# nikopj/FlashAttention.jl

Measured on AMD Instinct MI355X. Metric: effective attention TFLOP/s (fwd) at N=4096,d=64; % of bf16 MFMA peak, higher is better.
Workload: dtype bf16; 1 GPU; configs[1]: dense_fa bf16 forward, (B,H,N,d)=(4,16,4096,64) per GPU; B=4, H=16, N=4096, d=64, slabs_per_gpu=64, global_batch_heads=64, parallelism=shard(B*H) x1, no collective

## Files before the change

### flashattention.jl_amd/csrc/fa_fwd.hip

```cpp
#include <type_traits>

#include "fa_common.h"
#include "fa_internal.h"
#include "fa_fwd_params.h"
#include "../../include/fa_hip.h"

#ifndef FA_FWD_STAMP
#define FA_FWD_STAMP(k)
#endif
#ifndef FA_FWD_ABL
#define FA_FWD_ABL 0
#endif
#ifndef FA_FWD_OAUX
#define FA_FWD_OAUX 0
#endif

namespace fa {

thread_local int g_fwd_variant = 0;
thread_local int g_fwd_last_path = 0;
thread_local float g_fwd_rescale_log2 = kRescaleLog2;


constexpr int kBM = 128;
constexpr int kBN = 64;
constexpr int kThreads = 256;

template <class T>
__device__ __forceinline__ u32x4 load_chunk(const T* base, int row, int col0, int nrows,
                                            int ncols, bool fast) {
    constexpr int EPC = 16 / sizeof(T);
    u32x4 z = {0u, 0u, 0u, 0u};
    if (row >= nrows) return z;
    const T* src = base + (int64_t)row * ncols;
    if (fast) {
        if (col0 >= ncols) return z;
        return *(const u32x4*)(src + col0);
    }
    union {
        T e[EPC];
        u32x4 v;
    } u;
#pragma unroll
    for (int e = 0; e < EPC; ++e) u.e[e] = (col0 + e < ncols) ? src[col0 + e] : (T)0.0f;
    return u.v;
}

template <class T, int D, int DV>
__global__ __launch_bounds__(kThreads) void dense_fwd_generic(FwdParams p) {
    typedef typename Frag8<T>::type F8;
    typedef typename Frag8<T>::half F4;
    constexpr int KROW = kBN * 2;
    constexpr int VROW = kBN * 2 + 16;
    constexpr int KCH = D * 8 / kThreads;
    constexpr int VCH = DV * 8 / kThreads;
    static_assert(KCH >= 1 && VCH >= 1, "head dim class too small");
    __shared__ __attribute__((aligned(16))) char smem[D * KROW + DV * VROW];
    char* const klds = smem;
    char* const vlds = smem + D * KROW;

    const int lid = xcd_remap(blockIdx.x, p.total_wg);
    const int b = lid / p.nqb;
    const int qb = lid - b * p.nqb;
    const int tid = threadIdx.x, lane = tid & 63, wave = tid >> 6;
    const int r = lane & 31, h = lane >> 5;
    const int N = p.N, Nk = p.Nk, d = p.d, dv = p.dv;
    const T* __restrict__ Qb = (const T*)p.Q + (int64_t)b * N * d;
    const T* __restrict__ Kb = (const T*)p.K + (int64_t)b * Nk * d;
    const T* __restrict__ Vb = (const T*)p.V + (int64_t)b * Nk * dv;
    const bool fast = p.fast != 0;

    const int qi = qb * kBM + wave * 32 + r;
    F8 qf[D / 16];
#pragma unroll
    for (int s = 0; s < D / 16; ++s)
#pragma unroll
        for (int e = 0; e < 8; ++e) {
            const int f = 16 * s + 8 * h + e;
            qf[s][e] = (qi < N && f < d) ? Qb[(int64_t)f * N + qi] : (T)0.0f;
        }

    const int g = lane >> 4, kh = g & 1, ii = lane & 15, qq = ii >> 2, pp = ii & 3;
    const int sig = (pp == 1) ? 2 : (pp == 2) ? 1 : pp;
    int koff[2];
#pragma unroll
    for (int kb = 0; kb < 2; ++kb)
        koff[kb] = (8 * h + qq) * KROW + (((kb * 2 + kh) ^ (((qq >> 1) & 1) << 1)) * 32) + 8 * sig;
    const int voff = r * VROW + 16 * h;

    f32x16 oacc[DV / 32];
#pragma unroll
    for (int cb = 0; cb < DV / 32; ++cb)
#pragma unroll
        for (int x = 0; x < 16; ++x) oacc[cb][x] = 0.0f;
    float m_run = kNegInf, l_run = 0.0f;
    const float c = p.scale_log2;

    u32x4 kreg[KCH], vreg[VCH];
    auto gload = [&](int j) {
        const int key0 = j * kBN;
#pragma unroll
        for (int it = 0; it < KCH; ++it) {
            const int ch = tid + kThreads * it;
            kreg[it] = load_chunk<T>(Kb, ch >> 3, key0 + (ch & 7) * 8, d, Nk, fast);
        }
#pragma unroll
        for (int it = 0; it < VCH; ++it) {
            const int ch = tid + kThreads * it;
            vreg[it] = load_chunk<T>(Vb, ch >> 3, key0 + (ch & 7) * 8, dv, Nk, fast);
        }
    };
    auto lstore = [&]() {
#pragma unroll
        for (int it = 0; it < KCH; ++it) {
            const int ch = tid + kThreads * it, f = ch >> 3, pc = ch & 7;
            const int off = f * KROW + (((pc >> 1) ^ (((f >> 1) & 1) << 1)) * 32) + (pc & 1) * 16;
            *(u32x4*)(klds + off) = kreg[it];
        }
#pragma unroll
        for (int it = 0; it < VCH; ++it) {
            const int ch = tid + kThreads * it;
            *(u32x4*)(vlds + (ch >> 3) * VROW + (ch & 7) * 16) = vreg[it];
        }
    };

    const int ntiles = (Nk + kBN - 1) / kBN;
    gload(0);
    lstore();
    __syncthreads();

    for (int j = 0; j < ntiles; ++j) {
        const bool more = j + 1 < ntiles;
        if (more) gload(j + 1);

        f32x16 sacc[2];
#pragma unroll
        for (int kb = 0; kb < 2; ++kb) {
#pragma unroll
            for (int x = 0; x < 16; ++x) sacc[kb][x] = 0.0f;
#pragma unroll
            for (int s = 0; s < D / 16; ++s) {
                const char* a = klds + koff[kb] + 16 * s * KROW;
                const F4 lo = __builtin_bit_cast(F4, ds_read_tr16(a));
                const F4 hi = __builtin_bit_cast(F4, ds_read_tr16(a + 4 * KROW));
                const F8 af = __builtin_shufflevector(lo, hi, 0, 1, 2, 3, 4, 5, 6, 7);
                sacc[kb] = mfma32x32x16(af, qf[s], sacc[kb]);
            }
        }

        const int key0 = j * kBN;
        if (key0 + kBN > Nk) {
#pragma unroll
            for (int kb = 0; kb < 2; ++kb)
#pragma unroll
                for (int x = 0; x < 16; ++x) {
                    const int kt = kb * 32 + (x & 3) + 4 * ((x >> 2) & 1) + 8 * h + 16 * (x >> 3);
                    if (key0 + kt >= Nk) sacc[kb][x] = kNegInf;
                }
        }

        float mt = kNegInf;
#pragma unroll
        for (int kb = 0; kb < 2; ++kb)
#pragma unroll
            for (int x = 0; x < 16; ++x) mt = fmaxf(mt, sacc[kb][x]);
        mt = swap_halves_max(mt);
        const float m_new = fmaxf(m_run, mt);
        const float alpha = exp2_fast((m_run - m_new) * c);
        const float mc = m_new * c;
        float ls = 0.0f;
        F8 pf[2][2];
#pragma unroll
        for (int kb = 0; kb < 2; ++kb)
#pragma unroll
            for (int x = 0; x < 16; ++x) {
                const float pv = exp2_fast(fmaf(sacc[kb][x], c, -mc));
                ls += pv;
                pf[kb][x >> 3][x & 7] = (T)pv;
            }
        l_run = l_run * alpha + ls;
        m_run = m_new;
#pragma unroll
        for (int cb = 0; cb < DV / 32; ++cb)
#pragma unroll
            for (int x = 0; x < 16; ++x) oacc[cb][x] *= alpha;

#pragma unroll
        for (int cb = 0; cb < DV / 32; ++cb)
#pragma unroll
            for (int kb = 0; kb < 2; ++kb)
#pragma unroll
                for (int s = 0; s < 2; ++s) {
                    const F8 va = *(const F8*)(vlds + voff + cb * 32 * VROW + (kb * 32 + 16 * s) * 2);
                    oacc[cb] = mfma32x32x16(va, pf[kb][s], oacc[cb]);
                }

        __syncthreads();
        if (more) {
            lstore();
            __syncthreads();
        }
    }

    const float lt = swap_halves_sum(l_run);
    const float inv = 1.0f / lt;
    if (qi < N) {
        T* Ob = (T*)p.O + (int64_t)b * N * dv;
#pragma unroll
        for (int cb = 0; cb < DV / 32; ++cb)
#pragma unroll
            for (int x = 0; x < 16; ++x) {
                const int cc = cb * 32 + acc_row(x, h);
                if (cc < dv) Ob[(int64_t)cc * N + qi] = (T)(oacc[cb][x] * inv);
            }
        if (h == 0) {
            p.m[(int64_t)b * N + qi] = m_run * p.scale;
            p.l[(int64_t)b * N + qi] = lt;
        }
    }
}

template <int D, int DV>
__global__ __launch_bounds__(kThreads) void dense_fwd_generic_f32(FwdParams p) {
    constexpr int KROWF = kBN;
    constexpr int VROWF = kBN + 1;
    constexpr int KCH = D * 16 / kThreads;
    constexpr int VCH = DV * 16 / kThreads;
    static_assert(KCH >= 1 && VCH >= 1, "head dim class too small");
    __shared__ __attribute__((aligned(16))) float smem[D * KROWF + DV * VROWF];
    float* const klds = smem;
    float* const vlds = smem + D * KROWF;

    const int lid = xcd_remap(blockIdx.x, p.total_wg);
    const int b = lid / p.nqb;
    const int qb = lid - b * p.nqb;
    const int tid = threadIdx.x, lane = tid & 63, wave = tid >> 6;
    const int r = lane & 31, h = lane >> 5;
    const int N = p.N, Nk = p.Nk, d = p.d, dv = p.dv;
    const float* __restrict__ Qb = (const float*)p.Q + (int64_t)b * N * d;
    const float* __restrict__ Kb = (const float*)p.K + (int64_t)b * Nk * d;
    const float* __restrict__ Vb = (const float*)p.V + (int64_t)b * Nk * dv;
    const bool fast = p.fast != 0;

    const int qi = qb * kBM + wave * 32 + r;
    float qf[D / 2];
#pragma unroll
    for (int t = 0; t < D / 2; ++t) {
        const int f = 2 * t + h;
        qf[t] = (qi < N && f < d) ? Qb[(int64_t)f * N + qi] : 0.0f;
    }

    f32x16 oacc[DV / 32];
#pragma unroll
    for (int cb = 0; cb < DV / 32; ++cb)
#pragma unroll
        for (int x = 0; x < 16; ++x) oacc[cb][x] = 0.0f;
    float m_run = kNegInf, l_run = 0.0f;
    const float c = p.scale_log2;

    u32x4 kreg[KCH], vreg[VCH];
    auto gload = [&](int j) {
        const int key0 = j * kBN;
#pragma unroll
        for (int it = 0; it < KCH; ++it) {
            const int ch = tid + kThreads * it;
            kreg[it] = load_chunk<float>(Kb, ch >> 4, key0 + (ch & 15) * 4, d, Nk, fast);
        }
#pragma unroll
        for (int it = 0; it < VCH; ++it) {
            const int ch = tid + kThreads * it;
            vreg[it] = load_chunk<float>(Vb, ch >> 4, key0 + (ch & 15) * 4, dv, Nk, fast);
        }
    };
    auto lstore = [&]() {
#pragma unroll
        for (int it = 0; it < KCH; ++it) {
            const int ch = tid + kThreads * it;
            *(u32x4*)(klds + (ch >> 4) * KROWF + (ch & 15) * 4) = kreg[it];
        }
#pragma unroll
        for (int it = 0; it < VCH; ++it) {
            const int ch = tid + kThreads * it;
            float* dst = vlds + (ch >> 4) * VROWF + (ch & 15) * 4;
#pragma unroll
            for (int e = 0; e < 4; ++e) dst[e] = __uint_as_float(vreg[it][e]);
        }
    };

    const int ntiles = (Nk + kBN - 1) / kBN;
    gload(0);
    lstore();
    __syncthreads();

    for (int j = 0; j < ntiles; ++j) {
        const bool more = j + 1 < ntiles;
        if (more) gload(j + 1);

        f32x16 sacc[2];
#pragma unroll
        for (int kb = 0; kb < 2; ++kb) {
#pragma unroll
            for (int x = 0; x < 16; ++x) sacc[kb][x] = 0.0f;
#pragma unroll
            for (int t = 0; t < D / 2; ++t)
                sacc[kb] = mfma32x32x2(klds[(2 * t + h) * KROWF + kb * 32 + r], qf[t], sacc[kb]);
        }

        const int key0 = j * kBN;
        if (key0 + kBN > Nk) {
#pragma unroll
            for (int kb = 0; kb < 2; ++kb)
#pragma unroll
                for (int x = 0; x < 16; ++x)
                    if (key0 + kb * 32 + acc_row(x, h) >= Nk) sacc[kb][x] = kNegInf;
        }

        float mt = kNegInf;
#pragma unroll
        for (int kb = 0; kb < 2; ++kb)
#pragma unroll
            for (int x = 0; x < 16; ++x) mt = fmaxf(mt, sacc[kb][x]);
        mt = swap_halves_max(mt);
        const float m_new = fmaxf(m_run, mt);
        const float alpha = exp2_fast((m_run - m_new) * c);
        const float mc = m_new * c;
        float ls = 0.0f;
#pragma unroll
        for (int kb = 0; kb < 2; ++kb)
#pragma unroll
            for (int x = 0; x < 16; ++x) {
                const float pv = exp2_fast(fmaf(sacc[kb][x], c, -mc));
                ls += pv;
                sacc[kb][x] = pv;
            }
        l_run = l_run * alpha + ls;
        m_run = m_new;
#pragma unroll
        for (int cb = 0; cb < DV / 32; ++cb)
#pragma unroll
            for (int x = 0; x < 16; ++x) oacc[cb][x] *= alpha;

#pragma unroll
        for (int cb = 0; cb < DV / 32; ++cb)
#pragma unroll
            for (int kb = 0; kb < 2; ++kb)
#pragma unroll
                for (int x = 0; x < 16; ++x)
                    oacc[cb] = mfma32x32x2(vlds[(cb * 32 + r) * VROWF + kb * 32 + acc_row(x, h)],
                                           sacc[kb][x], oacc[cb]);

        __syncthreads();
        if (more) {
            lstore();
            __syncthreads();
        }
    }

    const float lt = swap_halves_sum(l_run);
    const float inv = 1.0f / lt;
    if (qi < N) {
        float* Ob = (float*)p.O + (int64_t)b * N * dv;
#pragma unroll
        for (int cb = 0; cb < DV / 32; ++cb)
#pragma unroll
            for (int x = 0; x < 16; ++x) {
                const int cc = cb * 32 + acc_row(x, h);
                if (cc < dv) Ob[(int64_t)cc * N + qi] = oacc[cb][x] * inv;
            }
        if (h == 0) {
            p.m[(int64_t)b * N + qi] = m_run * p.scale;
            p.l[(int64_t)b * N + qi] = lt;
        }
    }
}


template <class T, int D, int DV, int NW, int BN, int NQB, bool SPLIT = false, bool WIDE = false>
__device__ __forceinline__ void dense_fwd_tiled(const FwdParams& p) {
    typedef typename Frag8<T>::type F8;
    typedef typename Frag8<T>::half F4;
    constexpr int NTH = 64 * NW;
    constexpr int BM = 32 * NW * NQB;
    constexpr int NKB = BN / 32;
    constexpr int KROW = BN * 2;
    constexpr int VROW = BN * 2 + 16;
    constexpr int KBYTES = D * KROW, VBYTES = DV * VROW, STAGE = KBYTES + VBYTES;
    constexpr int CPR = BN / 8;
    constexpr int KTOT = D * CPR, VTOT = DV * CPR;
    constexpr int KCH = (KTOT + NTH - 1) / NTH;
    constexpr int VCH = (VTOT + NTH - 1) / NTH;
    static_assert(KTOT % NTH == 0 || KTOT < NTH, "tile split");
    static_assert(VTOT % NTH == 0 || VTOT < NTH, "tile split");
    constexpr int ROWB = BM * 2;
    constexpr int QOOFF = (2 * STAGE + 16 + 255) & ~255;
    constexpr int QOB = WIDE ? (D > DV ? D : DV) * ROWB : 0;
    __shared__ __attribute__((aligned(256))) char smem[QOOFF + QOB];
    auto qo_at = [](int f, int byteoff) {
        const int X = (f & 3) | (((f >> 2) & 1) << 2);
        return f * ROWB + (((byteoff >> 5) ^ X) << 5) + (byteoff & 31);
    };
    char* const qoimg = smem + QOOFF;

    auto kswz = [](int f) { return BN == 64 ? (((f >> 1) & 1) << 1) : ((f & 3) << 1); };

    FA_FWD_STAMP(0);
    int lid = xcd_remap(blockIdx.x, p.total_wg);
    const int split = SPLIT ? lid % p.nsplit : 0;
    if (SPLIT) lid /= p.nsplit;
    const int b = lid / p.nqb;
    const int qb = lid - b * p.nqb;
    const int tid = threadIdx.x, lane = tid & 63, wave = tid >> 6;
    const int r = lane & 31, h = lane >> 5;
    const int N = p.N, Nk = p.Nk, d = p.d, dv = p.dv;
    const auto qrs = slab_rsrc((const T*)p.Q + (int64_t)b * N * d, (uint32_t)(N * d * (int)sizeof(T)));
    const int ldk = p.ldk;
    const auto krs = slab_rsrc((const T*)p.K + (int64_t)b * ldk * d, (uint32_t)(ldk * d * (int)sizeof(T)));
    const auto vrs = slab_rsrc((const T*)p.V + (int64_t)b * ldk * dv, (uint32_t)(ldk * dv * (int)sizeof(T)));

    int qiv[NQB];
    F8 qf[NQB][D / 16];
    if constexpr (WIDE) {
        static_assert(D * ROWB % (1024 * NW) == 0, "Q image DMA split");
#pragma unroll
        for (int it = 0; it < D * ROWB / 1024 / NW; ++it) {
            const int k = it * NW + wave;
            const int P = k * 1024 + lane * 16, f = P / ROWB, pb = P - f * ROWB;
            const int X = (f & 3) | (((f >> 2) & 1) << 2);
            const int lb = (((pb >> 5) ^ X) << 5) + (pb & 31);
            __builtin_amdgcn_raw_ptr_buffer_load_lds(qrs, (__attribute__((address_space(3))) void*)(qoimg + k * 1024), 16,
                                                     (f * N + qb * BM) * 2 + lb, 0, 0, 0);
        }
#pragma unroll
        for (int u = 0; u < NQB; ++u) qiv[u] = qb * BM + (wave * NQB + u) * 32 + r;
    }
#pragma unroll
    for (int u = 0; u < NQB && !WIDE; ++u) {
        qiv[u] = qb * BM + (wave * NQB + u) * 32 + r;
#pragma unroll
        for (int s = 0; s < D / 16; ++s)
#pragma unroll
            for (int e = 0; e < 8; ++e) {
                const int f = 16 * s + 8 * h + e;
                const unsigned short w = __builtin_amdgcn_raw_buffer_load_b16(qrs, (f * N + qiv[u]) * 2, 0, 0);
                qf[u][s][e] = __builtin_bit_cast(T, w);
            }
    }

    const int g = lane >> 4, kh = g & 1, ii = lane & 15, qq = ii >> 2, pp = ii & 3;
    const int sig = (pp == 1) ? 2 : (pp == 2) ? 1 : pp;
    int koff[NKB];
#pragma unroll
    for (int kb = 0; kb < NKB; ++kb)
        koff[kb] = (8 * h + qq) * KROW + (((kb * 2 + kh) ^ kswz(qq)) * 32) + 8 * sig;
    const int voff = r * VROW + 16 * h;

    int kgo[KCH], kso[KCH], vgo[VCH], vso[VCH];
    const bool kact = KTOT >= NTH || tid < KTOT, vact = VTOT >= NTH || tid < VTOT;
#pragma unroll
    for (int it = 0; it < KCH; ++it) {
        const int ch = tid + NTH * it, f = ch / CPR, pc = ch % CPR;
        kgo[it] = kact ? (f * ldk + pc * 8) * 2 : 0x7FFFFFF0;
        kso[it] = kact ? f * KROW + (((pc >> 1) ^ kswz(f)) * 32) + (pc & 1) * 16 : 2 * STAGE;
    }
#pragma unroll
    for (int it = 0; it < VCH; ++it) {
        const int ch = tid + NTH * it, f = ch / CPR, pc = ch % CPR;
        vgo[it] = vact ? (f * ldk + pc * 8) * 2 : 0x7FFFFFF0;
        vso[it] = vact ? f * VROW + pc * 16 : 2 * STAGE - KBYTES;
    }

    f32x16 oacc[NQB][DV / 32];
#pragma unroll
    for (int u = 0; u < NQB; ++u)
#pragma unroll
        for (int cb = 0; cb < DV / 32; ++cb)
#pragma unroll
            for (int x = 0; x < 16; ++x) oacc[u][cb][x] = 0.0f;
    float m_used[NQB], m_true[NQB], l_run[NQB];
#pragma unroll
    for (int u = 0; u < NQB; ++u) { m_used[u] = kNegInf; m_true[u] = kNegInf; l_run[u] = 0.0f; }
    const float c = p.scale_log2;
    const float thr_raw = p.rescale_log2 / c;
    const int NT = (Nk + BN - 1) / BN;
    const bool ragged = (Nk % BN) != 0;

    u32x4 kreg[KCH], vreg[VCH];
    auto gload = [&](int j) {
        const int kb0 = j * BN * 2;
#pragma unroll
        for (int it = 0; it < KCH; ++it) kreg[it] = __builtin_amdgcn_raw_buffer_load_b128(krs, kgo[it] + kb0, 0, 0);
#pragma unroll
        for (int it = 0; it < VCH; ++it) vreg[it] = __builtin_amdgcn_raw_buffer_load_b128(vrs, vgo[it] + kb0, 0, 0);
    };
    auto lstore = [&](char* buf, int j) {
        if (ragged && j == NT - 1) {
#pragma unroll
            for (int it = 0; it < VCH; ++it) {
                const int ch = tid + NTH * it;
                if (j * BN + (ch % CPR) * 8 >= Nk) vreg[it] = u32x4{0u, 0u, 0u, 0u};
            }
        }
#pragma unroll
        for (int it = 0; it < KCH; ++it) *(u32x4*)((kact ? buf : smem) + kso[it]) = kreg[it];
#pragma unroll
        for (int it = 0; it < VCH; ++it) *(u32x4*)((vact ? buf : smem) + KBYTES + vso[it]) = vreg[it];
    };

    auto compute = [&](const char* klds, const char* vlds, int j) {
        f32x16 sacc[NQB][NKB];
#pragma unroll
        for (int kb = 0; kb < NKB; ++kb) {
#pragma unroll
            for (int u = 0; u < NQB; ++u)
#pragma unroll
                for (int x = 0; x < 16; ++x) sacc[u][kb][x] = 0.0f;
#pragma unroll
            for (int s = 0; s < D / 16; ++s) {
                const char* a = klds + koff[kb] + 16 * s * KROW;
                const F4 lo = __builtin_bit_cast(F4, ds_read_tr16(a));
                const F4 hi = __builtin_bit_cast(F4, ds_read_tr16(a + 4 * KROW));
                const F8 af = __builtin_shufflevector(lo, hi, 0, 1, 2, 3, 4, 5, 6, 7);
#pragma unroll
                for (int u = 0; u < NQB; ++u) sacc[u][kb] = mfma32x32x16(af, qf[u][s], sacc[u][kb]);
            }
        }
        if (ragged && j == NT - 1) {
            const int key0 = j * BN;
#pragma unroll
            for (int u = 0; u < NQB; ++u)
#pragma unroll
                for (int kb = 0; kb < NKB; ++kb)
#pragma unroll
                    for (int x = 0; x < 16; ++x) {
                        const int kt = kb * 32 + (x & 3) + 4 * ((x >> 2) & 1) + 8 * h + 16 * (x >> 3);
                        if (key0 + kt >= Nk) sacc[u][kb][x] = kNegInf;
                    }
        }
        F8 pf[NQB][NKB][2];
#pragma unroll
        for (int u = 0; u < NQB; ++u) {
            const float mt = (FA_FWD_ABL & 4) ? sacc[u][0][0] : lane_max<NKB>(sacc[u]);
            m_true[u] = vmax(m_true[u], mt);
            if (__builtin_amdgcn_ballot_w64(mt > m_used[u] + thr_raw) != 0) {
                const float m_new = fmaxf(m_used[u], swap_halves_max(mt));
                const float alpha = exp2_fast((m_used[u] - m_new) * c);
                l_run[u] *= alpha;
#pragma unroll
                for (int cb = 0; cb < DV / 32; ++cb)
#pragma unroll
                    for (int x = 0; x < 16; ++x) oacc[u][cb][x] *= alpha;
                m_used[u] = m_new;
            }
            const float mc = m_used[u] * c;
            float ps[4];
#pragma unroll
            for (int kb = 0; kb < NKB; ++kb)
#pragma unroll
                for (int x = 0; x < 16; ++x) {
                    const float arg = fmaf(sacc[u][kb][x], c, -mc);
                    const float pv = (FA_FWD_ABL & 1) ? arg : exp2_fast(arg);
                    if (kb == 0 && x < 4) ps[x] = pv; else if (!(FA_FWD_ABL & 2)) ps[x & 3] += pv;
                    pf[u][kb][x >> 3][x & 7] = (T)pv;
                }
            l_run[u] += (ps[0] + ps[1]) + (ps[2] + ps[3]);
        }
#pragma unroll
        for (int cb = 0; cb < DV / 32; ++cb)
#pragma unroll
            for (int kb = 0; kb < NKB; ++kb)
#pragma unroll
                for (int s = 0; s < 2; ++s) {
                    const F8 va = *(const F8*)(vlds + voff + cb * 32 * VROW + (kb * 32 + 16 * s) * 2);
#pragma unroll
                    for (int u = 0; u < NQB; ++u) oacc[u][cb] = mfma32x32x16(va, pf[u][kb][s], oacc[u][cb]);
                }
    };

    char* const buf0 = smem;
    char* const buf1 = smem + STAGE;
    const int jt0 = SPLIT ? split * p.tps : 0, jt1 = SPLIT ? min(NT, jt0 + p.tps) : NT;
    gload(jt0);
    lstore(buf0, jt0);
    if constexpr (WIDE) asm volatile("s_waitcnt vmcnt(0)" ::: "memory");
    __syncthreads();
    if constexpr (WIDE) {
#pragma unroll
        for (int u = 0; u < NQB; ++u)
#pragma unroll
            for (int s = 0; s < D / 16; ++s) {
                const int tb = ((wave * NQB + u) * 32 + 16 * kh + 4 * pp) * 2;
                const F4 lo = __builtin_bit_cast(F4, ds_read_tr16(qoimg + qo_at(16 * s + 8 * h + qq, tb)));
                const F4 hi = __builtin_bit_cast(F4, ds_read_tr16(qoimg + qo_at(16 * s + 8 * h + 4 + qq, tb)));
                qf[u][s] = __builtin_shufflevector(lo, hi, 0, 1, 2, 3, 4, 5, 6, 7);
            }
    }
    FA_FWD_STAMP(1);
    for (int j = jt0; j < jt1; j += 2) {
        gload(min(j + 1, jt1 - 1));
        compute(buf0, buf0 + KBYTES, j);
        lstore(buf1, min(j + 1, jt1 - 1));
        __syncthreads();
        if (j + 1 < jt1) {
            gload(min(j + 2, jt1 - 1));
            compute(buf1, buf1 + KBYTES, j + 1);
            lstore(buf0, min(j + 2, jt1 - 1));
            __syncthreads();
        }
    }
    FA_FWD_STAMP(2);
#pragma unroll
    for (int u = 0; u < NQB; ++u) m_true[u] = swap_halves_max(m_true[u]);

    if constexpr (SPLIT) {
        const int64_t sb = (int64_t)split * p.batch + b;
#pragma unroll
        for (int u = 0; u < NQB; ++u) {
            const int qi = qiv[u];
            const float sc = exp2_fast((m_used[u] - m_true[u]) * c);
            const float lt = swap_halves_sum(l_run[u]) * sc;
            if (qi < N) {
                float* Op = p.opart + sb * N * dv;
#pragma unroll
                for (int cb = 0; cb < DV / 32; ++cb)
#pragma unroll
                    for (int x = 0; x < 16; ++x) {
                        const int cc = cb * 32 + acc_row(x, h);
                        if (cc < dv) Op[(int64_t)cc * N + qi] = oacc[u][cb][x] * sc;
                    }
                if (h == 0) {
                    p.mpart[sb * N + qi] = m_true[u];
                    p.lpart[sb * N + qi] = lt;
                }
            }
        }
        return;
    }

    if constexpr (WIDE) {
#pragma unroll
        for (int u = 0; u < NQB; ++u) {
            const int qi = qiv[u];
            const float lt = swap_halves_sum(l_run[u]);
            const float inv = 1.0f / lt;
            const int tb = ((wave * NQB + u) * 32 + r) * 2;
#pragma unroll
            for (int cb = 0; cb < DV / 32; ++cb)
#pragma unroll
                for (int x = 0; x < 16; ++x)
                    *(T*)(qoimg + qo_at(cb * 32 + acc_row(x, h), tb)) = (T)(oacc[u][cb][x] * inv);
            if (qi < N && h == 0) {
                p.m[(int64_t)b * N + qi] = m_true[u] * p.scale;
                p.l[(int64_t)b * N + qi] = lt * exp2_fast((m_used[u] - m_true[u]) * c);
            }
        }
        __syncthreads();
        const auto ors = slab_rsrc((T*)p.O + (int64_t)b * N * dv, (uint32_t)(N * dv * (int)sizeof(T)));
        constexpr int CPRO = ROWB / 16;
        static_assert(DV * CPRO % NTH == 0, "O image store split");
#pragma unroll
        for (int it = 0; it < DV * CPRO / NTH; ++it) {
            const int ch = it * NTH + tid, f = ch / CPRO, lb = (ch - f * CPRO) * 16;
            const int q = qb * BM + lb / 2;
            const u32x4 v4 = *(const u32x4*)(qoimg + qo_at(f, lb));
            const int off = (f < dv && q < N) ? (f * N + q) * 2 : 0x7FFFFFF0;
            __builtin_amdgcn_raw_buffer_store_b128(v4, ors, off, 0, FA_FWD_OAUX);
        }
        FA_FWD_STAMP(3);
        return;
    }
#pragma unroll
    for (int u = 0; u < NQB; ++u) {
        const int qi = qiv[u];
        const float lt = swap_halves_sum(l_run[u]);
        const float inv = 1.0f / lt;
        if (qi < N) {
            T* Ob = (T*)p.O + (int64_t)b * N * dv;
#pragma unroll
            for (int cb = 0; cb < DV / 32; ++cb)
#pragma unroll
                for (int x = 0; x < 16; ++x) {
                    const int cc = cb * 32 + acc_row(x, h);
                    if (cc < dv) Ob[(int64_t)cc * N + qi] = (T)(oacc[u][cb][x] * inv);
                }
            if (h == 0) {
                p.m[(int64_t)b * N + qi] = m_true[u] * p.scale;
                p.l[(int64_t)b * N + qi] = lt * exp2_fast((m_used[u] - m_true[u]) * c);
            }
        }
    }
}

template <class T, int D, int DV>
__global__ __launch_bounds__(512, 1) void dense_fwd_w8b64(FwdParams p) { dense_fwd_tiled<T, D, DV, 8, 64, 1>(p); }
template <class T, int D, int DV>
__global__ __launch_bounds__(512, 1) void dense_fwd_w8q2(FwdParams p) { dense_fwd_tiled<T, D, DV, 8, 64, 2>(p); }
template <class T, int D, int DV>
__global__ __launch_bounds__(512, 1) void dense_fwd_w8q2_wide(FwdParams p) {
    dense_fwd_tiled<T, D, DV, 8, 64, 2, false, (D <= 64 && DV <= 64)>(p);
}
template <class T, int D, int DV>
__global__ __launch_bounds__(512, 1) void dense_fwd_w8b64_wide(FwdParams p) { dense_fwd_tiled<T, D, DV, 8, 64, 1, false, true>(p); }
template <class T, int D, int DV>
__global__ __launch_bounds__(512, 1) void dense_fwd_w8q2_split(FwdParams p) { dense_fwd_tiled<T, D, DV, 8, 64, 2, true>(p); }
template <class T, int D, int DV>
__global__ __launch_bounds__(512, 1) void dense_fwd_w8b64_split(FwdParams p) { dense_fwd_tiled<T, D, DV, 8, 64, 1, true>(p); }

template <class T>
__global__ __launch_bounds__(256) void fwd_split_combine(FwdParams p, int64_t total) {
    const int64_t e = (int64_t)blockIdx.x * 256 + threadIdx.x;
    if (e >= total) return;
    const int N = p.N, dv = p.dv, B = p.batch;
    const int n = (int)(e % N);
    const int64_t rest = e / N;
    const int cc = (int)(rest % dv);
    const int b = (int)(rest / dv);
    const float c = p.scale_log2;
    float mx = kNegInf;
    for (int sp = 0; sp < p.nsplit; ++sp) mx = vmax(mx, p.mpart[((int64_t)sp * B + b) * N + n]);
    float L = 0.0f, acc = 0.0f;
    for (int sp = 0; sp < p.nsplit; ++sp) {
        const int64_t sb = (int64_t)sp * B + b;
        const float w = exp2_fast((p.mpart[sb * N + n] - mx) * c);
        L = fmaf(p.lpart[sb * N + n], w, L);
        acc = fmaf(p.opart[(sb * dv + cc) * N + n], w, acc);
    }
    ((T*)p.O)[((int64_t)b * dv + cc) * N + n] = (T)(acc / L);
    if (cc == 0) {
        p.m[(int64_t)b * N + n] = mx * p.scale;
        p.l[(int64_t)b * N + n] = L;
    }
}

struct SplitPlan {
    int nsplit = 1, tps = 0;
    size_t bytes = 0;
};
static SplitPlan split_plan(int dtype, int64_t N, int64_t Nk, int64_t d, int64_t dv, int64_t batch) {
    SplitPlan sp;
    const int Dc = head_dim_class(d), DVc = head_dim_class(dv);
    if (dtype == FA_DTYPE_F32 || dtype == FA_DTYPE_F64 || !Dc || !DVc) return sp;
    const int64_t rows = (Dc <= 64 && DVc <= 64) ? 512 : 256;
    const int64_t wgs = (N + rows - 1) / rows * batch;
    const int64_t NT = (Nk + kBN - 1) / kBN;
    if (wgs >= 256 || NT < 4) return sp;
    int64_t ns = std::min<int64_t>((512 + wgs - 1) / wgs, NT / 2);
    if (ns < 2) return sp;
    const int64_t tps = (NT + ns - 1) / ns;
    ns = (NT + tps - 1) / tps;
    if (ns < 2 || ns * wgs > INT32_MAX) return sp;
    sp.nsplit = (int)ns;
    sp.tps = (int)tps;
    auto al = [](size_t x) { return (x + 255) & ~(size_t)255; };
    sp.bytes = al((size_t)(ns * batch * N * dv) * 4) + 2 * al((size_t)(ns * batch * N) * 4) + 256;
    return sp;
}

bool launch_dense_fwd_p4(const FwdParams& p, int Dc, int DVc, int dtype, hipStream_t s, hipError_t* err);

template <class T, int D>
static hipError_t launch_dv(const FwdParams& p, int DVc, dim3 grid, hipStream_t s) {
    if (p.fast && (g_fwd_variant == 30 || (g_fwd_variant == 0 && D == 128 && DVc == 128))) {
        hipError_t e = hipSuccess;
        if (launch_dense_fwd_p4(p, D, DVc, std::is_same<T, bf16>::value ? FA_DTYPE_BF16 : FA_DTYPE_F16, s, &e)) {
            g_fwd_last_path = 30;
            return e;
        }
    }
    if (p.fast) {
        int v = g_fwd_variant;
        const bool wide = p.wide && (v == 0 || v == 5 || v == 7 || v == 30);
        if (v == 0 || v == 20 || v == 30) v = (D <= 64 && DVc <= 64) ? 7 : 5;
        const int nw = 8;
        const int rows = v == 7 ? 512 : 256;
        FwdParams q = p;
        q.nqb = (q.N + rows - 1) / rows;
        q.total_wg = q.nqb * (int)(p.total_wg / p.nqb) * (q.nsplit > 1 ? q.nsplit : 1);
        const dim3 g2((unsigned)q.total_wg);
        const dim3 blk(64 * nw);
#define FA_LAUNCH_T(KER)                                                                \
        switch (DVc) {                                                                  \
            case 32: hipLaunchKernelGGL((KER<T, D, 32>), g2, blk, 0, s, q); break;      \
            case 64: hipLaunchKernelGGL((KER<T, D, 64>), g2, blk, 0, s, q); break;      \
            case 128: hipLaunchKernelGGL((KER<T, D, 128>), g2, blk, 0, s, q); break;    \
            default: return hipErrorInvalidValue;                                       \
        }
        if (q.nsplit > 1 && rows == 256) { FA_LAUNCH_T(dense_fwd_w8b64_split) }
        else if (q.nsplit > 1) { FA_LAUNCH_T(dense_fwd_w8q2_split) }
        else if (v == 5 && wide) { FA_LAUNCH_T(dense_fwd_w8b64_wide) }
        else if (v == 5) { FA_LAUNCH_T(dense_fwd_w8b64) }
        else if (wide) { FA_LAUNCH_T(dense_fwd_w8q2_wide) }
        else { FA_LAUNCH_T(dense_fwd_w8q2) }
#undef FA_LAUNCH_T
        if (q.nsplit > 1) {
            const int64_t total = (int64_t)q.N * q.dv * q.batch;
            hipLaunchKernelGGL(fwd_split_combine<T>, dim3((unsigned)((total + 255) / 256)), dim3(256), 0, s, q, total);
        }
        return hipGetLastError();
    }
    switch (DVc) {
        case 32: hipLaunchKernelGGL((dense_fwd_generic<T, D, 32>), grid, dim3(kThreads), 0, s, p); break;
        case 64: hipLaunchKernelGGL((dense_fwd_generic<T, D, 64>), grid, dim3(kThreads), 0, s, p); break;
        case 128: hipLaunchKernelGGL((dense_fwd_generic<T, D, 128>), grid, dim3(kThreads), 0, s, p); break;
        default: return hipErrorInvalidValue;
    }
    return hipGetLastError();
}
template <int D>
static hipError_t launch_dv_f32(const FwdParams& p, int DVc, dim3 grid, hipStream_t s) {
    switch (DVc) {
        case 32: hipLaunchKernelGGL((dense_fwd_generic_f32<D, 32>), grid, dim3(kThreads), 0, s, p); break;
        case 64: hipLaunchKernelGGL((dense_fwd_generic_f32<D, 64>), grid, dim3(kThreads), 0, s, p); break;
        case 128: hipLaunchKernelGGL((dense_fwd_generic_f32<D, 128>), grid, dim3(kThreads), 0, s, p); break;
        default: return hipErrorInvalidValue;
    }
    return hipGetLastError();
}
template <class T>
static hipError_t launch_typed(const FwdParams& p, int Dc, int DVc, dim3 grid, hipStream_t s) {
    switch (Dc) {
        case 32: return launch_dv<T, 32>(p, DVc, grid, s);
        case 64: return launch_dv<T, 64>(p, DVc, grid, s);
        case 128: return launch_dv<T, 128>(p, DVc, grid, s);
    }
    return hipErrorInvalidValue;
}
static hipError_t launch_f32(const FwdParams& p, int Dc, int DVc, dim3 grid, hipStream_t s) {
    switch (Dc) {
        case 32: return launch_dv_f32<32>(p, DVc, grid, s);
        case 64: return launch_dv_f32<64>(p, DVc, grid, s);
        case 128: return launch_dv_f32<128>(p, DVc, grid, s);
    }
    return hipErrorInvalidValue;
}

static bool aligned16(const void* ptr) { return ((uintptr_t)ptr & 15u) == 0; }

static bool fwd_pad_fits(int dtype, int64_t Nk, int64_t d, int64_t dv, int64_t batch) {
    const int64_t nk8 = (Nk + 7) / 8 * 8;
    return dtype != FA_DTYPE_F32 && dtype != FA_DTYPE_F64 && nk8 * d * 2 < INT32_MAX && nk8 * dv * 2 < INT32_MAX &&
           nk8 * (d > dv ? d : dv) * batch < ((int64_t)1 << 40);
}
static bool fwd_pad_needed(int dtype, int64_t Nk, int64_t d, int64_t dv, int64_t batch) {
    return Nk % 8 != 0 && fwd_pad_fits(dtype, Nk, d, dv, batch);
}
static size_t fwd_pad_bytes_any(int64_t Nk, int64_t d, int64_t dv, int64_t batch) {
    const int64_t nk8 = (Nk + 7) / 8 * 8;
    auto al = [](size_t x) { return (x + 255) & ~(size_t)255; };
    return al((size_t)(nk8 * d * batch) * 2) + al((size_t)(nk8 * dv * batch) * 2) + 256;
}
static size_t fwd_pad_bytes(int dtype, int64_t Nk, int64_t d, int64_t dv, int64_t batch) {
    if (!fwd_pad_needed(dtype, Nk, d, dv, batch)) return 0;
    return fwd_pad_bytes_any(Nk, d, dv, batch);
}
size_t dense_fwd_workspace(int dtype, int64_t N, int64_t Nk, int64_t d, int64_t dv, int64_t batch) {
    return fwd_pad_bytes(dtype, Nk, d, dv, batch) + split_plan(dtype, N, Nk, d, dv, batch).bytes;
}
template <class T>
__global__ __launch_bounds__(256) void fwd_pad_keys(const T* __restrict__ src, T* __restrict__ dst, int N, int Np,
                                                    int64_t total) {
    const int64_t e = (int64_t)blockIdx.x * 256 + threadIdx.x;
    if (e >= total) return;
    const int n = (int)(e % Np);
    const int64_t cb = e / Np;
    dst[e] = n < N ? src[cb * N + n] : (T)0.0f;
}

int launch_dense_fwd(const DenseArgs& a, hipStream_t s, const char** why) {
    g_fwd_last_path = 0;
    if (a.dtype == FA_DTYPE_F64) return launch_dense_fwd_f64(a, s, why);
    const int Dc = head_dim_class(a.d), DVc = head_dim_class(a.dv);
    if (!Dc || !DVc) {
        *why = "head dimension exceeds the compiled maximum (128)";
        return FA_ERR_UNSUPPORTED;
    }
    if (a.N > INT32_MAX / 2 || a.Nk > INT32_MAX / 2 || a.N * a.d > INT32_MAX ||
        a.Nk * a.d > INT32_MAX || a.Nk * a.dv > INT32_MAX || a.N * a.dv > INT32_MAX) {
        *why = "per-slab extent exceeds 2^31 elements";
        return FA_ERR_UNSUPPORTED;
    }
    FwdParams p;
    p.Q = a.Q; p.K = a.K; p.V = a.V; p.O = a.O; p.l = a.l; p.m = a.m;
    p.N = (int)a.N; p.Nk = (int)a.Nk; p.d = (int)a.d; p.dv = (int)a.dv;
    p.nqb = (int)((a.N + kBM - 1) / kBM);
    const int64_t total = (int64_t)p.nqb * a.batch;
    if (total > INT32_MAX) {
        *why = "grid too large";
        return FA_ERR_UNSUPPORTED;
    }
    p.total_wg = (int)total;
    p.scale = a.scale;
    p.scale_log2 = a.scale * kLog2e;
    p.rescale_log2 = g_fwd_rescale_log2;
    p.batch = (int)a.batch;
    p.nsplit = 1; p.tps = 0; p.opart = p.lpart = p.mpart = nullptr;
    const int epc = a.dtype == FA_DTYPE_F32 ? 4 : 8;
    p.ldk = (int)a.Nk;
    p.fast = (a.Nk % epc == 0) && aligned16(a.K) && aligned16(a.V);
    p.wide = a.N % 8 == 0 && aligned16(a.Q) && aligned16(a.O);
    size_t pad_bytes = 0;
    if (!p.fast && a.workspace && fwd_pad_fits(a.dtype, a.Nk, a.d, a.dv, a.batch) &&
        a.N * a.d * 2 < (int64_t)INT32_MAX &&
        a.workspace_bytes >= fwd_pad_bytes_any(a.Nk, a.d, a.dv, a.batch)) {
        pad_bytes = fwd_pad_bytes_any(a.Nk, a.d, a.dv, a.batch);
        const int64_t nk8 = (a.Nk + 7) / 8 * 8;
        char* w = (char*)(((uintptr_t)a.workspace + 255) & ~(uintptr_t)255);
        char* kp = w;
        char* vp = w + (((size_t)(nk8 * a.d * a.batch) * 2 + 255) & ~(size_t)255);
        const int64_t tk = nk8 * a.d * a.batch, tv = nk8 * a.dv * a.batch;
        if (a.dtype == FA_DTYPE_F16) {
            hipLaunchKernelGGL(fwd_pad_keys<f16>, dim3((unsigned)((tk + 255) / 256)), dim3(256), 0, s, (const f16*)a.K, (f16*)kp, (int)a.Nk, (int)nk8, tk);
            hipLaunchKernelGGL(fwd_pad_keys<f16>, dim3((unsigned)((tv + 255) / 256)), dim3(256), 0, s, (const f16*)a.V, (f16*)vp, (int)a.Nk, (int)nk8, tv);
        } else {
            hipLaunchKernelGGL(fwd_pad_keys<bf16>, dim3((unsigned)((tk + 255) / 256)), dim3(256), 0, s, (const bf16*)a.K, (bf16*)kp, (int)a.Nk, (int)nk8, tk);
            hipLaunchKernelGGL(fwd_pad_keys<bf16>, dim3((unsigned)((tv + 255) / 256)), dim3(256), 0, s, (const bf16*)a.V, (bf16*)vp, (int)a.Nk, (int)nk8, tv);
        }
        p.K = kp;
        p.V = vp;
        p.ldk = (int)nk8;
        p.fast = 1;
    }
    const int64_t esz = a.dtype == FA_DTYPE_F32 ? 4 : 2;
    if (a.N * a.d * esz >= (int64_t)INT32_MAX || (int64_t)p.ldk * a.d * esz >= (int64_t)INT32_MAX ||
        (int64_t)p.ldk * a.dv * esz >= (int64_t)INT32_MAX)
        p.fast = 0;
    const bool p4_fills = (g_fwd_variant == 30 || (g_fwd_variant == 0 && Dc == 128 && DVc == 128)) &&
                          (a.N + 255) / 256 * a.batch >= device_cus(s);
    if (p.fast && (g_fwd_variant == 0 || g_fwd_variant == 30) && !p4_fills && a.workspace) {
        const SplitPlan sp = split_plan(a.dtype, a.N, a.Nk, a.d, a.dv, a.batch);
        if (sp.nsplit > 1 && a.workspace_bytes >= pad_bytes + sp.bytes) {
            auto al = [](size_t x) { return (x + 255) & ~(size_t)255; };
            char* w = (char*)(((uintptr_t)a.workspace + 255) & ~(uintptr_t)255) + (pad_bytes ? pad_bytes - 256 : 0);
            w = (char*)(((uintptr_t)w + 255) & ~(uintptr_t)255);
            p.opart = (float*)w;
            w += al((size_t)(sp.nsplit * a.batch * a.N * a.dv) * 4);
            p.lpart = (float*)w;
            w += al((size_t)(sp.nsplit * a.batch * a.N) * 4);
            p.mpart = (float*)w;
            p.nsplit = sp.nsplit;
            p.tps = sp.tps;
        }
    }
    const dim3 grid((unsigned)total);
    hipError_t e;
    switch (a.dtype) {
        case FA_DTYPE_BF16: e = launch_typed<bf16>(p, Dc, DVc, grid, s); break;
        case FA_DTYPE_F16: e = launch_typed<f16>(p, Dc, DVc, grid, s); break;
        case FA_DTYPE_F32: e = launch_f32(p, Dc, DVc, grid, s); break;
        default: *why = "unknown dtype"; return FA_ERR_INVALID_ARG;
    }
    if (e != hipSuccess) {
        *why = hipGetErrorString(e);
        return FA_ERR_HIP;
    }
    return FA_OK;
}

}
```

Baseline: 1028 TFLOP/s.

## Prefetch first K/V tile early and pack O epilogue writes per-wave

Issues the first K/V global loads before the Q image DMA so their latency overlaps Q setup. Rewrites the WIDE epilogue to pack pairs of scaled outputs with DPP lane exchange and byte permute, so it does 32-bit LDS stores instead of 16-bit ones. Each wave now stores only its own slice of the O image to global memory, which lets a wave-level fence and barrier replace the block-wide __syncthreads. The early loads hold more registers live across Q setup, and the new epilogue is correct only if the per-wave ownership of the O image matches the layout exactly. Timing stamp hooks are added as well.

```diff
diff --git a/flashattention.jl_amd/csrc/fa_fwd.hip b/flashattention.jl_amd/csrc/fa_fwd.hip
--- a/flashattention.jl_amd/csrc/fa_fwd.hip
+++ b/flashattention.jl_amd/csrc/fa_fwd.hip
@@ -44,6 +44,19 @@
 #pragma unroll
     for (int e = 0; e < EPC; ++e) u.e[e] = (col0 + e < ncols) ? src[col0 + e] : (T)0.0f;
     return u.v;
+}
+
+template <class T>
+__device__ __forceinline__ unsigned pack_scaled(float a, float b, float s) {
+    if constexpr (std::is_same<T, f16>::value) {
+        unsigned r;
+        asm("v_fma_mixlo_f16 %0, %1, %3, 0\n\tv_fma_mixhi_f16 %0, %2, %3, 0" : "=&v"(r) : "v"(a), "v"(b), "v"(s));
+        return r;
+    } else {
+        typedef T T2 __attribute__((ext_vector_type(2)));
+        const T2 v = {(T)(a * s), (T)(b * s)};
+        return __builtin_bit_cast(unsigned, v);
+    }
 }
 
 template <class T, int D, int DV>
@@ -417,6 +430,33 @@
     const auto krs = slab_rsrc((const T*)p.K + (int64_t)b * ldk * d, (uint32_t)(ldk * d * (int)sizeof(T)));
     const auto vrs = slab_rsrc((const T*)p.V + (int64_t)b * ldk * dv, (uint32_t)(ldk * dv * (int)sizeof(T)));
 
+    const bool kact = KTOT >= NTH || tid < KTOT, vact = VTOT >= NTH || tid < VTOT;
+    int kgo[KCH], vgo[VCH];
+#pragma unroll
+    for (int it = 0; it < KCH; ++it) {
+        const int ch = tid + NTH * it, f = ch / CPR, pc = ch % CPR;
+        kgo[it] = kact ? (f * ldk + pc * 8) * 2 : 0x7FFFFFF0;
+    }
+#pragma unroll
+    for (int it = 0; it < VCH; ++it) {
+        const int ch = tid + NTH * it, f = ch / CPR, pc = ch % CPR;
+        vgo[it] = vact ? (f * ldk + pc * 8) * 2 : 0x7FFFFFF0;
+    }
+    const int NT = (Nk + BN - 1) / BN;
+    const bool ragged = (Nk % BN) != 0;
+    const int jt0 = SPLIT ? split * p.tps : 0, jt1 = SPLIT ? min(NT, jt0 + p.tps) : NT;
+
+    u32x4 kreg[KCH], vreg[VCH];
+    auto gload = [&](int j) {
+        const int kb0 = j * BN * 2;
+#pragma unroll
+        for (int it = 0; it < KCH; ++it) kreg[it] = __builtin_amdgcn_raw_buffer_load_b128(krs, kgo[it] + kb0, 0, 0);
+#pragma unroll
+        for (int it = 0; it < VCH; ++it) vreg[it] = __builtin_amdgcn_raw_buffer_load_b128(vrs, vgo[it] + kb0, 0, 0);
+    };
+    gload(jt0);
+    FA_FWD_STAMP(5);
+
     int qiv[NQB];
     F8 qf[NQB][D / 16];
     if constexpr (WIDE) {
@@ -432,6 +472,7 @@
         }
 #pragma unroll
         for (int u = 0; u < NQB; ++u) qiv[u] = qb * BM + (wave * NQB + u) * 32 + r;
+        FA_FWD_STAMP(4);
     }
 #pragma unroll
     for (int u = 0; u < NQB && !WIDE; ++u) {
@@ -454,18 +495,15 @@
         koff[kb] = (8 * h + qq) * KROW + (((kb * 2 + kh) ^ kswz(qq)) * 32) + 8 * sig;
     const int voff = r * VROW + 16 * h;
 
-    int kgo[KCH], kso[KCH], vgo[VCH], vso[VCH];
-    const bool kact = KTOT >= NTH || tid < KTOT, vact = VTOT >= NTH || tid < VTOT;
+    int kso[KCH], vso[VCH];
 #pragma unroll
     for (int it = 0; it < KCH; ++it) {
         const int ch = tid + NTH * it, f = ch / CPR, pc = ch % CPR;
-        kgo[it] = kact ? (f * ldk + pc * 8) * 2 : 0x7FFFFFF0;
         kso[it] = kact ? f * KROW + (((pc >> 1) ^ kswz(f)) * 32) + (pc & 1) * 16 : 2 * STAGE;
     }
 #pragma unroll
     for (int it = 0; it < VCH; ++it) {
         const int ch = tid + NTH * it, f = ch / CPR, pc = ch % CPR;
-        vgo[it] = vact ? (f * ldk + pc * 8) * 2 : 0x7FFFFFF0;
         vso[it] = vact ? f * VROW + pc * 16 : 2 * STAGE - KBYTES;
     }
 
@@ -481,17 +519,7 @@
     for (int u = 0; u < NQB; ++u) { m_used[u] = kNegInf; m_true[u] = kNegInf; l_run[u] = 0.0f; }
     const float c = p.scale_log2;
     const float thr_raw = p.rescale_log2 / c;
-    const int NT = (Nk + BN - 1) / BN;
-    const bool ragged = (Nk % BN) != 0;
-
-    u32x4 kreg[KCH], vreg[VCH];
-    auto gload = [&](int j) {
-        const int kb0 = j * BN * 2;
-#pragma unroll
-        for (int it = 0; it < KCH; ++it) kreg[it] = __builtin_amdgcn_raw_buffer_load_b128(krs, kgo[it] + kb0, 0, 0);
-#pragma unroll
-        for (int it = 0; it < VCH; ++it) vreg[it] = __builtin_amdgcn_raw_buffer_load_b128(vrs, vgo[it] + kb0, 0, 0);
-    };
+
     auto lstore = [&](char* buf, int j) {
         if (ragged && j == NT - 1) {
 #pragma unroll
@@ -578,11 +606,11 @@
 
     char* const buf0 = smem;
     char* const buf1 = smem + STAGE;
-    const int jt0 = SPLIT ? split * p.tps : 0, jt1 = SPLIT ? min(NT, jt0 + p.tps) : NT;
-    gload(jt0);
     lstore(buf0, jt0);
     if constexpr (WIDE) asm volatile("s_waitcnt vmcnt(0)" ::: "memory");
+    FA_FWD_STAMP(6);
     __syncthreads();
+    FA_FWD_STAMP(7);
     if constexpr (WIDE) {
 #pragma unroll
         for (int u = 0; u < NQB; ++u)
@@ -637,30 +665,46 @@
     }
 
     if constexpr (WIDE) {
+        const int odd = lane & 1;
+        const unsigned sel = odd ? 0x03020706u : 0x05040100u;
 #pragma unroll
         for (int u = 0; u < NQB; ++u) {
             const int qi = qiv[u];
             const float lt = swap_halves_sum(l_run[u]);
             const float inv = 1.0f / lt;
-            const int tb = ((wave * NQB + u) * 32 + r) * 2;
+            const int tb = ((wave * NQB + u) * 32 + (r & ~1)) * 2;
+            const int wb[2] = {qo_at(4 * h + 2 * odd, tb), qo_at(4 * h + 2 * odd + 1, tb)};
 #pragma unroll
             for (int cb = 0; cb < DV / 32; ++cb)
 #pragma unroll
-                for (int x = 0; x < 16; ++x)
-                    *(T*)(qoimg + qo_at(cb * 32 + acc_row(x, h), tb)) = (T)(oacc[u][cb][x] * inv);
+                for (int k = 0; k < 4; ++k)
+#pragma unroll
+                    for (int e = 0; e < 2; ++e) {
+                        const int x = 4 * k + e;
+                        const int ow = (int)pack_scaled<T>(oacc[u][cb][x], oacc[u][cb][x + 2], inv);
+                        const int nb = __builtin_amdgcn_mov_dpp(ow, 0xB1, 0xF, 0xF, true);
+                        *(unsigned*)(qoimg + wb[e] + (cb * 32 + 8 * k) * ROWB) =
+                            __builtin_amdgcn_perm((unsigned)nb, (unsigned)ow, sel);
+                    }
             if (qi < N && h == 0) {
                 p.m[(int64_t)b * N + qi] = m_true[u] * p.scale;
                 p.l[(int64_t)b * N + qi] = lt * exp2_fast((m_used[u] - m_true[u]) * c);
             }
         }
-        __syncthreads();
+        FA_FWD_STAMP(8);
+        __builtin_amdgcn_fence(__ATOMIC_ACQ_REL, "wavefront");
+        __builtin_amdgcn_wave_barrier();
+        FA_FWD_STAMP(9);
         const auto ors = slab_rsrc((T*)p.O + (int64_t)b * N * dv, (uint32_t)(N * dv * (int)sizeof(T)));
-        constexpr int CPRO = ROWB / 16;
-        static_assert(DV * CPRO % NTH == 0, "O image store split");
-#pragma unroll
-        for (int it = 0; it < DV * CPRO / NTH; ++it) {
-            const int ch = it * NTH + tid, f = ch / CPRO, lb = (ch - f * CPRO) * 16;
-            const int q = qb * BM + lb / 2;
+        constexpr int TPW = 32 * NQB, CPW = TPW / 8, RPI = 64 / CPW;
+        static_assert(DV % RPI == 0, "O image store split");
+        const int oc = lane % CPW, rs = lane / CPW;
+        const int fr = NQB == 2 ? ((rs & 1) | ((rs & 2) << 1) | ((rs & 4) >> 1)) : rs;
+        const int lb = (wave * TPW + oc * 8) * 2;
+        const int q = qb * BM + wave * TPW + oc * 8;
+#pragma unroll
+        for (int it = 0; it < DV / RPI; ++it) {
+            const int f = it * RPI + fr;
             const u32x4 v4 = *(const u32x4*)(qoimg + qo_at(f, lb));
             const int off = (f < dv && q < N) ? (f * N + q) * 2 : 0x7FFFFFF0;
             __builtin_amdgcn_raw_buffer_store_b128(v4, ors, off, 0, FA_FWD_OAUX);
```

Measured after the change: 1042 TFLOP/s, median of 6. 1.3% higher.
